# Coder-Yu/QRec

Measured on NVIDIA H100. Metric: BPR triples/sec at d=64, higher is better.
Workload: dtype f32

## Files before the change

qrec_b200/csrc/bpr_kernels.cu:

```cuda
#include <cmath>

#include "common.h"
#include "device.cuh"
#include "lane_shape.h"
#include "philox.cuh"
#include "bpr_step.cuh"
#include "um_waves.cuh"

namespace {

using namespace qrec;
using namespace qrec::bpr;

template <typename T, int E>
__global__ void __launch_bounds__(256)
bpr_sgd_ordered_kernel(T* __restrict__ P, T* __restrict__ Q, int d, long long n,
                       const int* __restrict__ u, const int* __restrict__ i,
                       const int* __restrict__ j, const int* __restrict__ wu,
                       const int* __restrict__ wi, const int* __restrict__ wj, int* ver_p,
                       int* ver_q, unsigned long long* ticket, T lr, T reg_u, T reg_i,
                       double* loss) {
  const int lane = threadIdx.x & 31;
  double local_loss = 0.0;
  const T a_u = mul_rn(lr, reg_u), a_i = mul_rn(lr, reg_i);
  while (true) {
    unsigned long long k = 0;
    if (lane == 0) k = atomicAdd(ticket, 1ULL);
    k = __shfl_sync(0xffffffffu, k, 0);
    if (k >= (unsigned long long)n) break;
    const int uu = u[k], ii = i[k], jj = j[k];
    const int* vp = lane == 0 ? ver_p + uu : (lane == 1 ? ver_q + ii : ver_q + jj);
    const int need = lane == 0 ? wu[k] : (lane == 1 ? wi[k] : wj[k]);
    unsigned backoff = 8, polls = 0;
    while (true) {
      const int have = lane < 3 ? ld_acquire_gpu(vp) : need;
      if (__all_sync(0xffffffffu, have == need)) break;
      __nanosleep(backoff);
      if (backoff < 64) backoff <<= 1;
      if (++polls > (1u << 27)) __trap();
    }
    T* pr = P + (size_t)uu * d;
    T* qir = Q + (size_t)ii * d;
    T* qjr = Q + (size_t)jj * d;
    T p[E], qi[E], qj[E];
    T di = 0, dj = 0;
#pragma unroll
    for (int e = 0; e < E; ++e) {
      const int c = e * 32 + lane;
      if (c < d) {
        p[e] = __ldcg(pr + c);
        qi[e] = __ldcg(qir + c);
        qj[e] = __ldcg(qjr + c);
        di += p[e] * qi[e];
        dj += p[e] * qj[e];
      } else {
        p[e] = qi[e] = qj[e] = 0;
      }
    }
    di = warp_sum(di);
    dj = warp_sum(dj);
    const T s = sigmoid_full(sub_rn(di, dj));
    const T g = mul_rn(lr, sub_rn((T)1, s));
#pragma unroll
    for (int e = 0; e < E; ++e) {
      const int c = e * 32 + lane;
      if (c < d) {
        T pn, qin, qjn;
        bpr_update_parity(p[e], qi[e], qj[e], g, a_u, a_i, pn, qin, qjn);
        __stcg(pr + c, pn);
        __stcg(qir + c, qin);
        __stcg(qjr + c, qjn);
      }
    }
    __threadfence();
    __syncwarp();
    if (lane < 3) red_release_gpu_add(const_cast<int*>(vp), 1);
    if (lane == 0) local_loss += neg_log(s);
  }
  if (lane == 0 && local_loss != 0.0) atomicAdd(loss, local_loss);
}

template <int LPR, int VPL, int UNROLL>
__global__ void __launch_bounds__(256)
bpr_sgd_batch_kernel(float* __restrict__ P, float* __restrict__ Q, int nvec, long long n,
                     const int* __restrict__ u, const int* __restrict__ i,
                     const int* __restrict__ j, float lr, float reg_u, float reg_i,
                     double* loss) {
  constexpr int TPW = 32 / LPR;
  const int lane = threadIdx.x & 31;
  const int sub = lane / LPR, l = lane % LPR;
  const long long warp = ((long long)blockIdx.x * blockDim.x + threadIdx.x) >> 5;
  const long long nwarps = ((long long)gridDim.x * blockDim.x) >> 5;
  const int d = nvec * 4;
  const float a_u = lr * reg_u, a_i = lr * reg_i;
  float lsum = 0.f;

  for (long long base = warp * 32; base < n; base += nwarps * 32) {
    const long long k = base + lane;
    int mu = 0, mi = 0, mj = 0;
    if (k < n) {
      mu = __ldg(u + k);
      mi = __ldg(i + k);
      mj = __ldg(j + k);
    }
    const int cnt = (n - base) < 32 ? (int)(n - base) : 32;
    for (int s0 = 0; s0 < cnt; s0 += TPW * UNROLL) {
      float4 p[UNROLL][VPL], qi[UNROLL][VPL], qj[UNROLL][VPL];
      float* pr[UNROLL];
      float* qir[UNROLL];
      float* qjr[UNROLL];
      bool ok[UNROLL];
#pragma unroll
      for (int r = 0; r < UNROLL; ++r) {
        const int t = s0 + r * TPW + sub;
        const int uu = __shfl_sync(0xffffffffu, mu, t & 31);
        const int ii = __shfl_sync(0xffffffffu, mi, t & 31);
        const int jj = __shfl_sync(0xffffffffu, mj, t & 31);
        ok[r] = t < cnt;
        pr[r] = P + (size_t)uu * d + l * 4;
        qir[r] = Q + (size_t)ii * d + l * 4;
        qjr[r] = Q + (size_t)jj * d + l * 4;
#pragma unroll
        for (int v = 0; v < VPL; ++v) {
          if (ok[r] && (l + v * LPR) < nvec) {
            p[r][v] = *reinterpret_cast<const float4*>(pr[r] + v * LPR * 4);
            qi[r][v] = *reinterpret_cast<const float4*>(qir[r] + v * LPR * 4);
            qj[r][v] = *reinterpret_cast<const float4*>(qjr[r] + v * LPR * 4);
          } else {
            p[r][v] = qi[r][v] = qj[r][v] = make_float4(0.f, 0.f, 0.f, 0.f);
          }
        }
      }
#pragma unroll
      for (int r = 0; r < UNROLL; ++r) {
        float x = 0.f;
#pragma unroll
        for (int v = 0; v < VPL; ++v) x += dot4(p[r][v], qi[r][v]) - dot4(p[r][v], qj[r][v]);
        x = group_sum<LPR>(x);
        const float s = fast_sigmoid(x);
        const float g = lr * (1.0f - s);
        if (ok[r]) {
          if (l == 0) lsum += fast_neg_log(s);
#pragma unroll
          for (int v = 0; v < VPL; ++v) {
            if ((l + v * LPR) < nvec) {
              float4 dp, dqi, dqj;
              bpr_step4(p[r][v], qi[r][v], qj[r][v], g, a_u, a_i, dp, dqi, dqj);
              red_add_v4(pr[r] + v * LPR * 4, dp);
              red_add_v4(qir[r] + v * LPR * 4, dqi);
              red_add_v4(qjr[r] + v * LPR * 4, dqj);
            }
          }
        }
      }
    }
  }
  block_add_loss(lsum, loss);
}


template <int LPR>
__global__ void __launch_bounds__(256)
bpr_sgd_staged_kernel(float* __restrict__ P, int nvec, long long n, const int* __restrict__ u,
                      const int* __restrict__ pos_i, const int* __restrict__ pos_j,
                      const float* __restrict__ R, float* __restrict__ D, float lr, float reg_u,
                      float reg_i, double* loss) {
  constexpr int TPW = 32 / LPR;
  const int lane = threadIdx.x & 31;
  const int sub = lane / LPR, l = lane % LPR;
  const long long group = (((long long)blockIdx.x * blockDim.x + threadIdx.x) >> 5) * TPW + sub;
  const long long ngroups = (((long long)gridDim.x * blockDim.x) >> 5) * TPW;
  const int d = nvec * 4;
  const float a_u = lr * reg_u, a_i = lr * reg_i;
  float lsum = 0.f;
  const long long rounds = (n + ngroups - 1) / ngroups;
  for (long long it = 0; it < rounds; ++it) {
    const long long k = it * ngroups + group;
    const bool ok = k < n && l < nvec;
    float4 p = make_float4(0.f, 0.f, 0.f, 0.f), qi = p, qj = p;
    float* pr = nullptr;
    size_t oi = 0, oj = 0;
    if (ok) {
      pr = P + (size_t)__ldg(u + k) * d + l * 4;
      oi = (size_t)__ldg(pos_i + k) * d + l * 4;
      oj = (size_t)__ldg(pos_j + k) * d + l * 4;
      p = *reinterpret_cast<const float4*>(pr);
      qi = __ldg(reinterpret_cast<const float4*>(R + oi));
      qj = __ldg(reinterpret_cast<const float4*>(R + oj));
    }
    float x = dot4(p, qi) - dot4(p, qj);
    x = group_sum<LPR>(x);
    const float s = fast_sigmoid(x);
    const float g = lr * (1.0f - s);
    if (ok) {
      if (l == 0) lsum += fast_neg_log(s);
      float4 dp, dqi, dqj;
      bpr_step4(p, qi, qj, g, a_u, a_i, dp, dqi, dqj);
      red_add_v4(pr, dp);
      *reinterpret_cast<float4*>(D + oi) = dqi;
      *reinterpret_cast<float4*>(D + oj) = dqj;
    }
  }
  block_add_loss(lsum, loss);
}


template <int UNROLL, int TMA_MASK>
__global__ void __launch_bounds__(256)
bpr_sgd_batch_tma_kernel(float* __restrict__ P, float* __restrict__ Q, long long n,
                         const int* __restrict__ u, const int* __restrict__ i,
                         const int* __restrict__ j, float lr, float reg_u, float reg_i,
                         double* loss) {
  constexpr int LPR = 16, TPW = 2, D = 64;
  constexpr int ROWS = ((TMA_MASK >> 0) & 1) + ((TMA_MASK >> 1) & 1) + ((TMA_MASK >> 2) & 1);
  constexpr int SLOT_P = 0, SLOT_I = (TMA_MASK & 1), SLOT_J = (TMA_MASK & 1) + ((TMA_MASK >> 1) & 1);
  constexpr int SLOT_FLOATS = UNROLL * TPW * ROWS * D;
  extern __shared__ __align__(128) float stage[];
  const int lane = threadIdx.x & 31, wib = threadIdx.x >> 5;
  const int sub = lane / LPR, l = lane % LPR;
  const long long warp = ((long long)blockIdx.x * blockDim.x + threadIdx.x) >> 5;
  const long long nwarps = ((long long)gridDim.x * blockDim.x) >> 5;
  const float a_u = lr * reg_u, a_i = lr * reg_i;
  float* my_stage = stage + (size_t)wib * 2 * SLOT_FLOATS;
  float lsum = 0.f;
  int buf = 0;

  for (long long base = warp * 32; base < n; base += nwarps * 32) {
    const long long k = base + lane;
    int mu = 0, mi = 0, mj = 0;
    if (k < n) {
      mu = __ldg(u + k);
      mi = __ldg(i + k);
      mj = __ldg(j + k);
    }
    const int cnt = (n - base) < 32 ? (int)(n - base) : 32;
    for (int s0 = 0; s0 < cnt; s0 += TPW * UNROLL) {
      float4 p[UNROLL], qi[UNROLL], qj[UNROLL];
      int uu[UNROLL], ii[UNROLL], jj[UNROLL];
      bool ok[UNROLL];
#pragma unroll
      for (int r = 0; r < UNROLL; ++r) {
        const int t = s0 + r * TPW + sub;
        uu[r] = __shfl_sync(0xffffffffu, mu, t & 31);
        ii[r] = __shfl_sync(0xffffffffu, mi, t & 31);
        jj[r] = __shfl_sync(0xffffffffu, mj, t & 31);
        ok[r] = t < cnt;
        if (ok[r]) {
          p[r] = *reinterpret_cast<const float4*>(P + (size_t)uu[r] * D + l * 4);
          qi[r] = *reinterpret_cast<const float4*>(Q + (size_t)ii[r] * D + l * 4);
          qj[r] = *reinterpret_cast<const float4*>(Q + (size_t)jj[r] * D + l * 4);
        } else {
          p[r] = qi[r] = qj[r] = make_float4(0.f, 0.f, 0.f, 0.f);
        }
      }
      if (l < 3) asm volatile("cp.async.bulk.wait_group.read 1;" ::: "memory");
      __syncwarp();
      float* slot = my_stage + (size_t)buf * SLOT_FLOATS;
#pragma unroll
      for (int r = 0; r < UNROLL; ++r) {
        float x = dot4(p[r], qi[r]) - dot4(p[r], qj[r]);
        x = group_sum<LPR>(x);
        const float s = fast_sigmoid(x);
        const float g = lr * (1.0f - s);
        if (ok[r]) {
          if (l == 0) lsum += fast_neg_log(s);
          float4 dp, dqi, dqj;
          bpr_step4(p[r], qi[r], qj[r], g, a_u, a_i, dp, dqi, dqj);
          float* trip = slot + (size_t)(r * TPW + sub) * ROWS * D;
          if (TMA_MASK & 1) *reinterpret_cast<float4*>(trip + SLOT_P * D + l * 4) = dp;
          else red_add_v4(P + (size_t)uu[r] * D + l * 4, dp);
          if (TMA_MASK & 2) *reinterpret_cast<float4*>(trip + SLOT_I * D + l * 4) = dqi;
          else red_add_v4(Q + (size_t)ii[r] * D + l * 4, dqi);
          if (TMA_MASK & 4) *reinterpret_cast<float4*>(trip + SLOT_J * D + l * 4) = dqj;
          else red_add_v4(Q + (size_t)jj[r] * D + l * 4, dqj);
        }
      }
      asm volatile("fence.proxy.async.shared::cta;" ::: "memory");
      __syncwarp();
      if (l < 3 && ((TMA_MASK >> l) & 1)) {
        const int srow = (l == 0) ? SLOT_P : (l == 1 ? SLOT_I : SLOT_J);
#pragma unroll
        for (int r = 0; r < UNROLL; ++r) {
          if (ok[r]) {
            float* dst = (l == 0) ? (P + (size_t)uu[r] * D) : (Q + (size_t)(l == 1 ? ii[r] : jj[r]) * D);
            const float* src = slot + (size_t)(r * TPW + sub) * ROWS * D + srow * D;
            asm volatile("cp.reduce.async.bulk.global.shared::cta.bulk_group.add.f32 [%0], [%1], %2;" ::"l"(dst),
                         "r"((uint32_t)__cvta_generic_to_shared(src)), "n"(D * 4)
                         : "memory");
          }
        }
        asm volatile("cp.async.bulk.commit_group;" ::: "memory");
      }
      buf ^= 1;
    }
  }
  if (l < 3) asm volatile("cp.async.bulk.wait_group 0;" ::: "memory");
  block_add_loss(lsum, loss);
}


constexpr int UM_STAGE_FLOATS = 2 * 4 * 64;
constexpr int UM_STAGE_GROUPS = 16;
constexpr int UM_STAGE_SMEM = UM_STAGE_GROUPS * 2 * (UM_STAGE_FLOATS * 4 + 8);

__device__ __forceinline__ void bulk_row_load(float* smem_dst, const float* gsrc, uint64_t* bar) {
  asm volatile("cp.async.bulk.shared::cluster.global.mbarrier::complete_tx::bytes [%0], [%1], 256, [%2];"
               ::"r"(smem_u32(smem_dst)), "l"(gsrc), "r"(smem_u32(bar)) : "memory");
}

template <int LPR, int G, bool FULL, bool SAMPLE, bool SIG, bool TMA>
__device__ __forceinline__ void
usermajor_epoch(float* __restrict__ P, float* __restrict__ Q, const float* __restrict__ Qr, int nvec, long long n,
                const int* __restrict__ wave_user, const long long* __restrict__ rowptr, const int* __restrict__ i,
                const int* __restrict__ j, float lr, float reg_u, float reg_i, double* loss, FusedSampler fs,
                long long trip_off, const uint32_t* __restrict__ rated_sig) {
  static_assert(!TMA || (LPR == 16 && G == 4 && FULL), "the TMA fetch is laid out for d = 64, G = 4");
  constexpr int GPW = 32 / LPR;
  const int lane = threadIdx.x & 31;
  const int sub = lane / LPR, l = lane % LPR;
  const unsigned gmask = (LPR == 32) ? 0xffffffffu : (((1u << LPR) - 1u) << (sub * LPR));
  const int group = (int)((blockIdx.x * blockDim.x + threadIdx.x) >> 5) * GPW + sub;
  const int ngroups = (int)((gridDim.x * blockDim.x) >> 5) * GPW;
  const int d = FULL ? LPR * 4 : nvec * 4;
  const bool act = FULL ? true : (l < nvec);
  const float a_u = lr * reg_u, a_i = lr * reg_i;
  const float one_m_au = 1.0f - a_u, one_m_ai = 1.0f - a_i;
  float lsum = 0.f;
  qrec::pdl_launch_dependents();
  bool waited = false;
  float* stage = nullptr;
  uint64_t* bar = nullptr;
  uint32_t phase0 = 0, phase1 = 0;
  if constexpr (TMA) {
    extern __shared__ __align__(128) unsigned char smem_raw[];
    float* stage_all = reinterpret_cast<float*>(smem_raw);
    uint64_t* bars = reinterpret_cast<uint64_t*>(stage_all + UM_STAGE_GROUPS * 2 * UM_STAGE_FLOATS);
    const int g_in_cta = (threadIdx.x >> 5) * GPW + sub;
    stage = stage_all + (size_t)g_in_cta * 2 * UM_STAGE_FLOATS;
    bar = bars + g_in_cta * 2;
    if (l == 0) { mbar_init(bar, 1); mbar_init(bar + 1, 1); }
    asm volatile("fence.mbarrier_init.release.cluster;" ::: "memory");
    asm volatile("fence.proxy.async.shared::cta;" ::: "memory");
    __syncthreads();
  }
  const int ub = __ldg(wave_user + 1);
  for (int uu = __ldg(wave_user) + group; uu < ub; uu += ngroups) {
    long long lo = __ldg(rowptr + uu) - trip_off, hi = __ldg(rowptr + uu + 1) - trip_off;
    lo = lo > 0 ? lo : 0;
    hi = hi < n ? hi : n;
    if (lo >= hi) continue;
    float* prow = P + (size_t)uu * d + l * 4;
    float4 p = act ? *reinterpret_cast<const float4*>(prow) : make_float4(0.f, 0.f, 0.f, 0.f);
    long long rated_lo = 0, rated_hi = 0;
    if (SAMPLE) {
      rated_lo = __ldg(fs.rated_rowptr + uu);
      rated_hi = __ldg(fs.rated_rowptr + uu + 1);
    }
    for (long long base = lo; base < hi; base += LPR) {
      const int m = (hi - base) < LPR ? (int)(hi - base) : LPR;
      int mi = 0, mj = 0;
      if (l < m) {
        mi = __ldg(i + base + l);
        if (SAMPLE) {
          if (SIG)
            mj = qrec::sample_negative_sig(base + l + trip_off, fs.epoch, fs.seed_lo, fs.seed_hi, fs.num_items,
                                           fs.rated_cols, rated_lo, rated_hi,
                                           rated_sig + (size_t)uu * qrec::RATED_SIG_WORDS);
          else
            mj = qrec::sample_negative(base + l + trip_off, fs.epoch, fs.seed_lo, fs.seed_hi, fs.num_items, fs.rated_cols,
                                       rated_lo, rated_hi);
        } else {
          mj = __ldg(j + base + l);
        }
      }
      if (!waited) {
        qrec::pdl_wait();
        waited = true;
      }
      if (SAMPLE && l < m && fs.j_out != nullptr) fs.j_out[base + l] = mj;
      auto issue = [&](int t0) {
        const int src = sub * LPR + ((t0 + (l >> 1)) & (LPR - 1));
        const int idi = __shfl_sync(gmask, mi, src), idj = __shfl_sync(gmask, mj, src);
        const int rows_now = 2 * ((m - t0) < G ? (m - t0) : G);
        uint64_t* bb = bar + ((t0 / G) & 1);
        if (l == 0) mbar_expect_tx(bb, 256u * rows_now);
        __syncwarp(gmask);
        if (l < rows_now) bulk_row_load(stage + ((t0 / G) & 1) * UM_STAGE_FLOATS + l * 64, Qr + (size_t)((l & 1) ? idj : idi) * d, bb);
      };
      if constexpr (TMA) issue(0);
      for (int t0 = 0; t0 < m; t0 += G) {
        const float* slot = nullptr;
        if constexpr (TMA) {
          if (t0 + G < m) issue(t0 + G);
          const int s = (t0 / G) & 1;
          mbar_wait(bar + s, s ? phase1 : phase0);
          if (s) phase1 ^= 1u; else phase0 ^= 1u;
          slot = stage + s * UM_STAGE_FLOATS;
        }
        float4 qi[G], qj[G];
        int ri[G], rj[G];
#pragma unroll
        for (int f = 0; f < G; ++f) {
          ri[f] = __shfl_sync(gmask, mi, sub * LPR + ((t0 + f) & (LPR - 1)));
          rj[f] = __shfl_sync(gmask, mj, sub * LPR + ((t0 + f) & (LPR - 1)));
          if (t0 + f < m && act) {
            if constexpr (TMA) {
              qi[f] = *reinterpret_cast<const float4*>(slot + (2 * f) * 64 + l * 4);
              qj[f] = *reinterpret_cast<const float4*>(slot + (2 * f + 1) * 64 + l * 4);
            } else {
              qi[f] = qrec::ldg_no_l1_v4(reinterpret_cast<const float4*>(Qr + (size_t)ri[f] * d + l * 4));
              qj[f] = qrec::ldg_no_l1_v4(reinterpret_cast<const float4*>(Qr + (size_t)rj[f] * d + l * 4));
            }
          } else {
            qi[f] = qj[f] = make_float4(0.f, 0.f, 0.f, 0.f);
          }
        }
        if constexpr (TMA) __syncwarp(gmask);
#pragma unroll
        for (int f = 0; f < G; ++f) {
          if (t0 + f < m) {
            float x = dot4(p, qi[f]) - dot4(p, qj[f]);
            x = group_sum<LPR>(x, gmask);
            const float s = fast_sigmoid(x);
            const float g = lr * (1.0f - s);
            if (l == 0) lsum += fast_neg_log(s);
            if (act) {
              float4 dqi, dqj;
              bpr_step4_inplace(p, qi[f], qj[f], g, one_m_au, g * one_m_ai, a_i, dqi, dqj);
              red_add_v4(Q + (size_t)ri[f] * d + l * 4, dqi);
              red_add_v4(Q + (size_t)rj[f] * d + l * 4, dqj);
            }
          }
        }
      }
    }
    if (act) {
      const float4 p0 = __ldcg(reinterpret_cast<const float4*>(prow));
      red_add_v4(prow, make_float4(p.x - p0.x, p.y - p0.y, p.z - p0.z, p.w - p0.w));
    }
  }
  if (!waited) qrec::pdl_wait();
  block_add_loss(lsum, loss);
}

template <int LPR, int G, bool FULL, bool SAMPLE, int MINB = 3, bool SIG = false>
__global__ void __launch_bounds__(256, MINB)
bpr_sgd_usermajor_kernel(float* __restrict__ P, float* __restrict__ Q, const float* __restrict__ Qr, int nvec, long long n,
                         const int* __restrict__ wave_user, const long long* __restrict__ rowptr,
                         const int* __restrict__ i, const int* __restrict__ j, float lr, float reg_u, float reg_i,
                         double* loss, FusedSampler fs, long long trip_off, const uint32_t* __restrict__ rated_sig) {
  usermajor_epoch<LPR, G, FULL, SAMPLE, SIG, false>(P, Q, Qr, nvec, n, wave_user, rowptr, i, j, lr, reg_u, reg_i, loss, fs,
                                                    trip_off, rated_sig);
}

__global__ void __launch_bounds__(256, 3)
bpr_sgd_usermajor_tma_kernel(float* __restrict__ P, float* __restrict__ Q, const float* __restrict__ Qr, int nvec,
                             long long n, const int* __restrict__ wave_user, const long long* __restrict__ rowptr,
                             const int* __restrict__ i, const int* __restrict__ j, float lr, float reg_u, float reg_i,
                             double* loss, FusedSampler fs, long long trip_off, const uint32_t* __restrict__ rated_sig) {
  usermajor_epoch<16, 4, true, true, false, true>(P, Q, Qr, nvec, n, wave_user, rowptr, i, j, lr, reg_u, reg_i, loss, fs,
                                                  trip_off, rated_sig);
}

using UserMajorKernel = decltype(&bpr_sgd_usermajor_tma_kernel);

template <int LPR>
UserMajorKernel usermajor_kernel(int nvec, bool sample, bool sig) {
  if (nvec != LPR)
    return sample ? bpr_sgd_usermajor_kernel<LPR, 4, false, true> : bpr_sgd_usermajor_kernel<LPR, 4, false, false>;
  if (sig) return bpr_sgd_usermajor_kernel<LPR, 2, true, true, 4, true>;
  return sample ? bpr_sgd_usermajor_kernel<LPR, 2, true, true, 4> : bpr_sgd_usermajor_kernel<LPR, 4, true, false>;
}

constexpr int UM_SNAPSHOT_THREADS = 512, UM_SNAPSHOT_CTAS_PER_SM = 4;
__global__ void __launch_bounds__(UM_SNAPSHOT_THREADS, UM_SNAPSHOT_CTAS_PER_SM)
um_snapshot_kernel(const float4* __restrict__ Q, float4* __restrict__ Qr, long long n4) {
  const unsigned long long keep = qrec::l2_policy_evict_last();
  qrec::pdl_wait();
  qrec::pdl_launch_dependents();
  const long long stride = (long long)gridDim.x * blockDim.x;
  long long k = (long long)blockIdx.x * blockDim.x + threadIdx.x;
  for (; k + 3 * stride < n4; k += 4 * stride) {
    float4 v[4];
#pragma unroll
    for (int r = 0; r < 4; ++r) v[r] = qrec::ld_stream_v4(Q + k + r * stride, keep);
#pragma unroll
    for (int r = 0; r < 4; ++r) qrec::st_hint_v4(Qr + k + r * stride, v[r], keep);
  }
  for (; k < n4; k += stride) qrec::st_hint_v4(Qr + k, qrec::ld_stream_v4(Q + k, keep), keep);
}

__global__ void __launch_bounds__(256)
um_wave_table_kernel(const long long* __restrict__ rowptr, int n_users, long long n, long long trip_off,
                     long long wave_chunks, long long nwaves, int* __restrict__ wave_user) {
  const long long w = (long long)blockIdx.x * blockDim.x + threadIdx.x;
  if (w <= nwaves) wave_user[w] = um_wave_first_user(rowptr, n_users, n, trip_off, wave_chunks, w);
}

__global__ void __launch_bounds__(256)
rated_signature_kernel(int n_users, const long long* __restrict__ rowptr, const int* __restrict__ cols,
                       uint32_t* __restrict__ sig) {
  const int lane = threadIdx.x & 31;
  const long long warp = ((long long)blockIdx.x * blockDim.x + threadIdx.x) >> 5;
  const long long nwarps = ((long long)gridDim.x * blockDim.x) >> 5;
  for (long long uu = warp; uu < n_users; uu += nwarps) {
    const long long lo = __ldg(rowptr + uu), hi = __ldg(rowptr + uu + 1);
    for (long long e = lo + lane; e < hi; e += 32) {
      const int c = __ldg(cols + e);
      atomicOr(sig + (size_t)uu * qrec::RATED_SIG_WORDS + ((c >> 5) & (qrec::RATED_SIG_WORDS - 1)), 1u << (c & 31));
    }
  }
}

template <typename T>
__global__ void __launch_bounds__(256)
sumsq_kernel(const T* __restrict__ x, long long n, double* out) {
  double acc = 0.0;
  const long long tid = (long long)blockIdx.x * blockDim.x + threadIdx.x;
  const long long stride = (long long)gridDim.x * blockDim.x;
  if constexpr (sizeof(T) == 4) {
    const long long n4 = n >> 2;
    const float4* x4 = reinterpret_cast<const float4*>(x);
    for (long long k = tid; k < n4; k += stride) {
      const float4 v = __ldg(x4 + k);
      acc += (double)v.x * v.x + (double)v.y * v.y + (double)v.z * v.z + (double)v.w * v.w;
    }
    for (long long k = (n4 << 2) + tid; k < n; k += stride) acc += (double)x[k] * x[k];
  } else {
    for (long long k = tid; k < n; k += stride) acc += (double)x[k] * (double)x[k];
  }
  acc = warp_sum(acc);
  __shared__ double wsum[8];
  if ((threadIdx.x & 31) == 0) wsum[threadIdx.x >> 5] = acc;
  __syncthreads();
  if (threadIdx.x == 0) {
    double t = 0.0;
    for (int w = 0; w < (int)(blockDim.x >> 5); ++w) t += wsum[w];
    atomicAdd(out, t);
  }
}

template <typename T>
int launch_ordered(T* P, T* Q, int d, long long n, const int* u, const int* i, const int* j,
                   const int* wu, const int* wi, const int* wj, int* ver_p, int* ver_q,
                   unsigned long long* ticket, T lr, T reg_u, T reg_i, double* loss,
                   int n_warps, cudaStream_t st) {
  QREC_REQUIRE(P && Q && loss && ticket && ver_p && ver_q, "bpr_sgd_ordered: null pointer");
  QREC_REQUIRE(d >= 1 && d <= 256, "bpr_sgd_ordered: d=%d unsupported (1..256)", d);
  QREC_REQUIRE(n >= 0, "bpr_sgd_ordered: n < 0");
  if (n == 0) return QREC_OK;
  QREC_REQUIRE(u && i && j && wu && wi && wj, "bpr_sgd_ordered: null index pointer");
  const int grid = n_warps > 0 ? capped_grid((n_warps + 7) / 8, 2) : sm_count() * 2;
  with_lane_elems(d, [&](auto e) {
    bpr_sgd_ordered_kernel<T, decltype(e)::E><<<grid, 256, 0, st>>>(P, Q, d, n, u, i, j, wu, wi, wj, ver_p, ver_q,
                                                                    ticket, lr, reg_u, reg_i, loss);
  });
  QREC_LAUNCH_CHECK();
  return QREC_OK;
}

}

namespace qrec {
int launch_bpr_batch(float* P, float* Q, int d, long long n, const int* u, const int* i,
                     const int* j, float lr, float reg_u, float reg_i, double* loss,
                     cudaStream_t st) {
  QREC_REQUIRE(P && Q && loss, "bpr_sgd_batch: null pointer");
  QREC_REQUIRE(d >= 4 && d <= 256 && (d % 4) == 0, "bpr_sgd_batch: d=%d unsupported (multiple of 4, 4..256)", d);
  QREC_REQUIRE(n >= 0, "bpr_sgd_batch: n < 0");
  if (n == 0) return QREC_OK;
  QREC_REQUIRE(u && i && j, "bpr_sgd_batch: null index pointer");
  const int nvec = d / 4;
  const long long warps_needed = (n + 31) / 32;
  const int grid = capped_grid((warps_needed + 7) / 8, 8);
  with_row_shape<256>(nvec, [&](auto s) {
    using S = decltype(s);
    bpr_sgd_batch_kernel<S::LPR, S::VPL, S::UNROLL><<<grid, 256, 0, st>>>(P, Q, nvec, n, u, i, j, lr, reg_u, reg_i,
                                                                          loss);
  });
  QREC_LAUNCH_CHECK();
  return QREC_OK;
}
}

extern "C" {

int qrec_bpr_sgd_ordered_f32(float* P, float* Q, int32_t d, int64_t n, const int32_t* u,
                             const int32_t* i, const int32_t* j, const int32_t* wu,
                             const int32_t* wi, const int32_t* wj, int32_t* ver_p,
                             int32_t* ver_q, unsigned long long* ticket, float lr, float reg_u,
                             float reg_i, double* loss, int32_t n_warps, void* stream) {
  return launch_ordered<float>(P, Q, d, n, u, i, j, wu, wi, wj, ver_p, ver_q, ticket, lr, reg_u,
                               reg_i, loss, n_warps, (cudaStream_t)stream);
}

int qrec_bpr_sgd_ordered_f64(double* P, double* Q, int32_t d, int64_t n, const int32_t* u,
                             const int32_t* i, const int32_t* j, const int32_t* wu,
                             const int32_t* wi, const int32_t* wj, int32_t* ver_p,
                             int32_t* ver_q, unsigned long long* ticket, double lr,
                             double reg_u, double reg_i, double* loss, int32_t n_warps, void* stream) {
  return launch_ordered<double>(P, Q, d, n, u, i, j, wu, wi, wj, ver_p, ver_q, ticket, lr, reg_u,
                                reg_i, loss, n_warps, (cudaStream_t)stream);
}

int qrec_bpr_sgd_batch_f32(float* P, float* Q, int32_t d, int64_t n, const int32_t* u,
                           const int32_t* i, const int32_t* j, float lr, float reg_u,
                           float reg_i, double* loss, void* stream) {
  return qrec::launch_bpr_batch(P, Q, d, n, u, i, j, lr, reg_u, reg_i, loss, (cudaStream_t)stream);
}

int qrec_bpr_sgd_batch_tma_f32(float* P, float* Q, int32_t d, int64_t n, const int32_t* u,
                               const int32_t* i, const int32_t* j, float lr, float reg_u,
                               float reg_i, double* loss, void* stream) {
  QREC_REQUIRE(P && Q && loss, "qrec_bpr_sgd_batch_tma_f32: null pointer");
  QREC_REQUIRE(d == 64, "qrec_bpr_sgd_batch_tma_f32: only d=64 (got %d); use qrec_bpr_sgd_batch_f32", d);
  QREC_REQUIRE(n >= 0, "qrec_bpr_sgd_batch_tma_f32: n < 0");
  if (n == 0) return QREC_OK;
  QREC_REQUIRE(u && i && j, "qrec_bpr_sgd_batch_tma_f32: null index pointer");
  constexpr int UN = 4, MASK = 1;
  constexpr int smem = 8 * 2 * UN * 2 * 64 * 4;
  QREC_CUDA(allow_dynamic_smem((const void*)bpr_sgd_batch_tma_kernel<UN, MASK>, smem));
  const int grid = capped_grid(((n + 31) / 32 + 7) / 8, 2);
  bpr_sgd_batch_tma_kernel<UN, MASK><<<grid, 256, smem, (cudaStream_t)stream>>>(P, Q, n, u, i, j, lr, reg_u, reg_i, loss);
  QREC_LAUNCH_CHECK();
  return QREC_OK;
}

}

namespace qrec {
int launch_usermajor(float* P, float* Q, int32_t d, int32_t n_users, int64_t n, const int64_t* rowptr,
                     const int32_t* i, const int32_t* j, float lr, float reg_u, float reg_i, double* loss,
                     bool sample, const int64_t* rated_rowptr, const int32_t* rated_cols, int32_t num_items,
                     uint64_t seed, uint32_t epoch, int32_t* j_out, long long trip_off, cudaStream_t st,
                     const uint32_t* rated_sig, bool tma) {
  if (n <= 0) return QREC_OK;
  QREC_REQUIRE(num_items >= 1, "qrec user-major epoch: num_items=%d (the item table's rows) must be given", num_items);
  QREC_REQUIRE(!tma || (d == 64 && sample), "qrec user-major epoch: the TMA fetch needs d = 64 and fused sampling");
  FusedSampler fs = {reinterpret_cast<const long long*>(rated_rowptr), rated_cols, num_items, (uint32_t)seed,
                     (uint32_t)(seed >> 32), epoch, j_out};
  const int nvec = d / 4;
  const int lpr = row_lpr(nvec);
  const bool sig = sample && rated_sig != nullptr;
  const UserMajorKernel kernel =
      tma ? bpr_sgd_usermajor_tma_kernel
          : with_row_shape<128>(nvec, [&](auto s) { return usermajor_kernel<decltype(s)::LPR>(nvec, sample, sig); });
  const int smem = tma ? UM_STAGE_SMEM : 0;
  if (tma) QREC_CUDA(allow_dynamic_smem((const void*)kernel, smem));
  int occ = 3;
  if (cudaOccupancyMaxActiveBlocksPerMultiprocessor(&occ, kernel, 256, smem) != cudaSuccess || occ < 1) occ = 3;
  const long long per_block = 8 * (32 / lpr);
  const long long max_users = n < n_users ? n : n_users;
  const int grid = capped_grid((max_users + per_block - 1) / per_block, occ);
  const size_t q_bytes = (size_t)num_items * d * sizeof(float);
  const long long wave = um_wave_chunks(n, num_items, d);
  const long long nwaves = um_num_waves(n, wave);
  float* Qr = nullptr;
  int* wave_user = nullptr;
  QREC_CUDA(cudaMallocAsync(reinterpret_cast<void**>(&Qr), q_bytes, st));
  const int rc = [&]() -> int {
    QREC_CUDA(cudaMallocAsync(reinterpret_cast<void**>(&wave_user), sizeof(int) * (size_t)(nwaves + 1), st));
    um_wave_table_kernel<<<(unsigned)((nwaves + 256) / 256), 256, 0, st>>>(reinterpret_cast<const long long*>(rowptr), n_users,
                                                                          n, trip_off, wave, nwaves, wave_user);
    QREC_CUDA(cudaGetLastError());
    count_launch();
    cudaLaunchAttribute pdl;
    pdl.id = cudaLaunchAttributeProgrammaticStreamSerialization;
    pdl.val.programmaticStreamSerializationAllowed = 1;
    const auto launch = [&](auto* fn, dim3 g, dim3 b, size_t shm, bool chained, auto... args) {
      cudaLaunchConfig_t cfg = {};
      cfg.gridDim = g;
      cfg.blockDim = b;
      cfg.dynamicSmemBytes = shm;
      cfg.stream = st;
      cfg.attrs = chained ? &pdl : nullptr;
      cfg.numAttrs = chained ? 1 : 0;
      return cudaLaunchKernelEx(&cfg, fn, args...);
    };
    const long long n4 = (long long)(q_bytes / sizeof(float4));
    const int copy_grid = sm_count() * UM_SNAPSHOT_CTAS_PER_SM;
    for (long long w = 0; w < nwaves; ++w) {
      QREC_CUDA(launch(um_snapshot_kernel, dim3(copy_grid), dim3(UM_SNAPSHOT_THREADS), 0, w > 0,
                       reinterpret_cast<const float4*>(Q), reinterpret_cast<float4*>(Qr), n4));
      count_launch();
      QREC_CUDA(launch(kernel, dim3(grid), dim3(256), (size_t)smem, true, P, Q, static_cast<const float*>(Qr), nvec,
                       (long long)n, static_cast<const int*>(wave_user + w), reinterpret_cast<const long long*>(rowptr), i, j,
                       lr, reg_u, reg_i, loss, fs, trip_off, rated_sig));
      if (w + 1 < nwaves) count_launch();
    }
    return QREC_OK;
  }();
  if (wave_user != nullptr) QREC_CUDA(cudaFreeAsync(wave_user, st));
  QREC_CUDA(cudaFreeAsync(Qr, st));
  if (rc != QREC_OK) return rc;
  QREC_LAUNCH_CHECK();
  return QREC_OK;
}
}

extern "C" {

int qrec_bpr_sgd_usermajor_f32(float* P, float* Q, int32_t d, int32_t n_users, int64_t n, int32_t num_items,
                               const int64_t* rowptr, const int32_t* i, const int32_t* j, float lr, float reg_u, float reg_i,
                               double* loss, void* stream) {
  QREC_REQUIRE(P && Q && loss, "qrec_bpr_sgd_usermajor_f32: null pointer");
  QREC_REQUIRE(d >= 4 && d <= 128 && (d % 4) == 0, "qrec_bpr_sgd_usermajor_f32: d=%d unsupported (multiple of 4, 4..128)", d);
  QREC_REQUIRE(n_users >= 0 && n >= 0, "qrec_bpr_sgd_usermajor_f32: negative size");
  if (n_users == 0 || n == 0) return QREC_OK;
  QREC_REQUIRE(rowptr && i && j, "qrec_bpr_sgd_usermajor_f32: null index pointer");
  return qrec::launch_usermajor(P, Q, d, n_users, n, rowptr, i, j, lr, reg_u, reg_i, loss, false, nullptr, nullptr, num_items,
                                0, 0, nullptr, 0, (cudaStream_t)stream, nullptr, false);
}

int qrec_bpr_epoch_usermajor_f32(float* P, float* Q, int32_t d, int32_t n_users, int64_t n, const int64_t* rowptr,
                                 const int32_t* i, const int64_t* rated_rowptr, const int32_t* rated_cols,
                                 int32_t num_items, uint64_t seed, uint32_t epoch, int32_t* j_out, float lr,
                                 float reg_u, float reg_i, double* loss, void* stream) {
  QREC_REQUIRE(P && Q && loss, "qrec_bpr_epoch_usermajor_f32: null pointer");
  QREC_REQUIRE(d >= 4 && d <= 128 && (d % 4) == 0, "qrec_bpr_epoch_usermajor_f32: d=%d unsupported (multiple of 4, 4..128)", d);
  QREC_REQUIRE(n_users >= 0 && n >= 0 && num_items >= 1, "qrec_bpr_epoch_usermajor_f32: bad size");
  if (n_users == 0 || n == 0) return QREC_OK;
  QREC_REQUIRE(rowptr && i && rated_rowptr && rated_cols, "qrec_bpr_epoch_usermajor_f32: null index pointer");
  return qrec::launch_usermajor(P, Q, d, n_users, n, rowptr, i, nullptr, lr, reg_u, reg_i, loss, true, rated_rowptr,
                                rated_cols, num_items, seed, epoch, j_out, 0, (cudaStream_t)stream, nullptr, false);
}

int qrec_rated_signature_build(int32_t n_users, const int64_t* rated_rowptr, const int32_t* rated_cols,
                               uint32_t* sig, void* stream) {
  QREC_REQUIRE(n_users >= 0, "qrec_rated_signature_build: n_users < 0");
  if (n_users == 0) return QREC_OK;
  QREC_REQUIRE(rated_rowptr && rated_cols && sig, "qrec_rated_signature_build: null pointer");
  cudaStream_t st = (cudaStream_t)stream;
  QREC_CUDA(cudaMemsetAsync(sig, 0, (size_t)n_users * qrec::RATED_SIG_WORDS * sizeof(uint32_t), st));
  rated_signature_kernel<<<capped_grid(((long long)n_users + 7) / 8, 8), 256, 0, st>>>(n_users, reinterpret_cast<const long long*>(rated_rowptr),
                                                     rated_cols, sig);
  QREC_LAUNCH_CHECK();
  return QREC_OK;
}

int qrec_bpr_epoch_usermajor_sig_f32(float* P, float* Q, int32_t d, int32_t n_users, int64_t n, const int64_t* rowptr,
                                     const int32_t* i, const int64_t* rated_rowptr, const int32_t* rated_cols,
                                     const uint32_t* rated_sig, int32_t num_items, uint64_t seed, uint32_t epoch,
                                     int32_t* j_out, float lr, float reg_u, float reg_i, double* loss, void* stream) {
  QREC_REQUIRE(P && Q && loss, "qrec_bpr_epoch_usermajor_sig_f32: null pointer");
  QREC_REQUIRE(d == 16 || d == 32 || d == 64 || d == 128,
               "qrec_bpr_epoch_usermajor_sig_f32: d=%d unsupported (16, 32, 64 or 128); use qrec_bpr_epoch_usermajor_f32", d);
  QREC_REQUIRE(n_users >= 0 && n >= 0 && num_items >= 1, "qrec_bpr_epoch_usermajor_sig_f32: bad size");
  if (n_users == 0 || n == 0) return QREC_OK;
  QREC_REQUIRE(rowptr && i && rated_rowptr && rated_cols && rated_sig, "qrec_bpr_epoch_usermajor_sig_f32: null index pointer");
  return qrec::launch_usermajor(P, Q, d, n_users, n, rowptr, i, nullptr, lr, reg_u, reg_i, loss, true, rated_rowptr,
                                rated_cols, num_items, seed, epoch, j_out, 0, (cudaStream_t)stream, rated_sig, false);
}

int qrec_bpr_epoch_usermajor_tma_f32(float* P, float* Q, int32_t d, int32_t n_users, int64_t n, const int64_t* rowptr,
                                     const int32_t* i, const int64_t* rated_rowptr, const int32_t* rated_cols,
                                     int32_t num_items, uint64_t seed, uint32_t epoch, int32_t* j_out, float lr,
                                     float reg_u, float reg_i, double* loss, void* stream) {
  QREC_REQUIRE(P && Q && loss, "qrec_bpr_epoch_usermajor_tma_f32: null pointer");
  QREC_REQUIRE(d == 64, "qrec_bpr_epoch_usermajor_tma_f32: d=%d unsupported (64 only: one 256-byte bulk copy per row); use "
                        "qrec_bpr_epoch_usermajor_f32", d);
  QREC_REQUIRE(n_users >= 0 && n >= 0 && num_items >= 1, "qrec_bpr_epoch_usermajor_tma_f32: bad size");
  if (n_users == 0 || n == 0) return QREC_OK;
  QREC_REQUIRE(rowptr && i && rated_rowptr && rated_cols, "qrec_bpr_epoch_usermajor_tma_f32: null index pointer");
  QREC_REQUIRE((reinterpret_cast<uintptr_t>(Q) & 15) == 0, "qrec_bpr_epoch_usermajor_tma_f32: Q must be 16-byte aligned");
  return qrec::launch_usermajor(P, Q, d, n_users, n, rowptr, i, nullptr, lr, reg_u, reg_i, loss, true, rated_rowptr,
                                rated_cols, num_items, seed, epoch, j_out, 0, (cudaStream_t)stream, nullptr, true);
}

int qrec_bpr_sgd_staged_f32(float* P, int32_t d, int64_t n, const int32_t* u, const int32_t* pos_i,
                            const int32_t* pos_j, const float* R, float* D, float lr, float reg_u,
                            float reg_i, double* loss, void* stream) {
  QREC_REQUIRE(d >= 4 && d <= 128 && (d % 4) == 0, "qrec_bpr_sgd_staged_f32: d=%d unsupported (multiple of 4, 4..128)", d);
  QREC_REQUIRE(n >= 0, "qrec_bpr_sgd_staged_f32: n < 0");
  if (n == 0) return QREC_OK;
  QREC_REQUIRE(P && u && pos_i && pos_j && R && D && loss, "qrec_bpr_sgd_staged_f32: null pointer");
  const int nvec = d / 4;
  cudaStream_t st = (cudaStream_t)stream;
  with_row_shape<128>(nvec, [&](auto s) {
    constexpr int LPR = decltype(s)::LPR;
    const long long per_block = 8 * (32 / LPR);
    const int grid = capped_grid((n + per_block - 1) / per_block, 8);
    bpr_sgd_staged_kernel<LPR><<<grid, 256, 0, st>>>(P, nvec, n, u, pos_i, pos_j, R, D, lr, reg_u, reg_i, loss);
  });
  QREC_LAUNCH_CHECK();
  return QREC_OK;
}

int qrec_sumsq_f32(const float* x, int64_t n, double* out, void* stream) {
  QREC_REQUIRE(out && (x || n == 0) && n >= 0, "qrec_sumsq_f32: bad argument");
  if (n == 0) return QREC_OK;
  QREC_REQUIRE((reinterpret_cast<uintptr_t>(x) & 15) == 0, "qrec_sumsq_f32: x not 16-byte aligned");
  sumsq_kernel<float><<<capped_grid((n / 4 + 255) / 256 + 1, 8), 256, 0, (cudaStream_t)stream>>>(x, n, out);
  QREC_LAUNCH_CHECK();
  return QREC_OK;
}

int qrec_table_snapshot_f32(const float* src, float* dst, int64_t n, void* stream) {
  QREC_REQUIRE(n >= 0 && (n % 4) == 0, "qrec_table_snapshot_f32: n=%lld must be a multiple of 4", (long long)n);
  if (n == 0) return QREC_OK;
  QREC_REQUIRE(src && dst, "qrec_table_snapshot_f32: null pointer");
  QREC_REQUIRE(((reinterpret_cast<uintptr_t>(src) | reinterpret_cast<uintptr_t>(dst)) & 15) == 0,
               "qrec_table_snapshot_f32: src and dst must be 16-byte aligned");
  um_snapshot_kernel<<<sm_count() * UM_SNAPSHOT_CTAS_PER_SM, UM_SNAPSHOT_THREADS, 0, (cudaStream_t)stream>>>(reinterpret_cast<const float4*>(src),
                                                                                 reinterpret_cast<float4*>(dst), n / 4);
  QREC_LAUNCH_CHECK();
  return QREC_OK;
}

int qrec_sumsq_f64(const double* x, int64_t n, double* out, void* stream) {
  QREC_REQUIRE(out && (x || n == 0) && n >= 0, "qrec_sumsq_f64: bad argument");
  if (n == 0) return QREC_OK;
  sumsq_kernel<double><<<capped_grid((n + 255) / 256, 8), 256, 0, (cudaStream_t)stream>>>(x, n, out);
  QREC_LAUNCH_CHECK();
  return QREC_OK;
}

}
```

qrec_b200/csrc/device.cuh:

```cuda
#pragma once
#include <cstdint>

namespace qrec {

__device__ __forceinline__ void red_add_v4(float* addr, float4 v) {
  asm volatile("red.global.add.v4.f32 [%0], {%1, %2, %3, %4};" ::"l"(addr), "f"(v.x), "f"(v.y), "f"(v.z), "f"(v.w) : "memory");
}

__device__ __forceinline__ unsigned long long l2_policy_evict_last() {
  unsigned long long pol;
  asm volatile("createpolicy.fractional.L2::evict_last.b64 %0, 1.0;" : "=l"(pol));
  return pol;
}
__device__ __forceinline__ float4 ld_stream_v4(const float4* p, unsigned long long pol) {
  float4 v;
  asm volatile("ld.global.nc.L1::no_allocate.L2::cache_hint.v4.f32 {%0, %1, %2, %3}, [%4], %5;"
               : "=f"(v.x), "=f"(v.y), "=f"(v.z), "=f"(v.w) : "l"(p), "l"(pol));
  return v;
}
__device__ __forceinline__ void st_hint_v4(float4* p, float4 v, unsigned long long pol) {
  asm volatile("st.global.L2::cache_hint.v4.f32 [%0], {%1, %2, %3, %4}, %5;" ::"l"(p), "f"(v.x), "f"(v.y), "f"(v.z), "f"(v.w),
               "l"(pol) : "memory");
}
__device__ __forceinline__ float4 ldg_no_l1_v4(const float4* p) {
  float4 v;
  asm volatile("ld.global.nc.L1::no_allocate.v4.f32 {%0, %1, %2, %3}, [%4];"
               : "=f"(v.x), "=f"(v.y), "=f"(v.z), "=f"(v.w) : "l"(p));
  return v;
}

__device__ __forceinline__ void pdl_wait() { asm volatile("griddepcontrol.wait;" ::: "memory"); }
__device__ __forceinline__ void pdl_launch_dependents() { asm volatile("griddepcontrol.launch_dependents;" ::: "memory"); }

__device__ __forceinline__ float dot4(float4 a, float4 b) { return a.x * b.x + a.y * b.y + a.z * b.z + a.w * b.w; }

__device__ __forceinline__ void fma4(float4& acc, float s, float4 x) {
  acc.x = fmaf(s, x.x, acc.x); acc.y = fmaf(s, x.y, acc.y);
  acc.z = fmaf(s, x.z, acc.z); acc.w = fmaf(s, x.w, acc.w);
}

template <typename T>
__device__ __forceinline__ T warp_sum(T v) {
#pragma unroll
  for (int o = 16; o > 0; o >>= 1) v += __shfl_xor_sync(0xffffffffu, v, o);
  return v;
}

template <int LPR>
__device__ __forceinline__ float group_sum(float v, unsigned mask = 0xffffffffu) {
#pragma unroll
  for (int o = LPR / 2; o > 0; o >>= 1) v += __shfl_xor_sync(mask, v, o);
  return v;
}

__device__ __forceinline__ float fast_sigmoid(float x) { return __fdividef(1.0f, 1.0f + __expf(-x)); }
__device__ __forceinline__ float fast_neg_log(float s) { return -__logf(s); }

__device__ __forceinline__ int ld_acquire_gpu(const int* p) {
  int v;
  asm volatile("ld.acquire.gpu.global.s32 %0, [%1];" : "=r"(v) : "l"(p) : "memory");
  return v;
}
__device__ __forceinline__ void red_release_gpu_add(int* p, int v) {
  asm volatile("red.release.gpu.global.add.s32 [%0], %1;" ::"l"(p), "r"(v) : "memory");
}

__device__ __forceinline__ void block_add_loss(float lsum, double* loss) {
  __shared__ float wsum[8];
  lsum = warp_sum(lsum);
  if ((threadIdx.x & 31) == 0) wsum[threadIdx.x >> 5] = lsum;
  __syncthreads();
  if (threadIdx.x == 0) {
    double t = 0.0;
    for (int w = 0; w < (int)(blockDim.x >> 5); ++w) t += (double)wsum[w];
    if (t != 0.0) atomicAdd(loss, t);
  }
}

__device__ __forceinline__ uint32_t smem_u32(const void* p) { return (uint32_t)__cvta_generic_to_shared(p); }

__device__ __forceinline__ void mbar_init(uint64_t* bar, uint32_t count) {
  asm volatile("mbarrier.init.shared::cta.b64 [%0], %1;" ::"r"(smem_u32(bar)), "r"(count));
}
__device__ __forceinline__ void mbar_expect_tx(uint64_t* bar, uint32_t bytes) {
  asm volatile("mbarrier.arrive.expect_tx.shared::cta.b64 _, [%0], %1;" ::"r"(smem_u32(bar)), "r"(bytes) : "memory");
}
__device__ __forceinline__ void mbar_arrive(uint64_t* bar) {
  asm volatile("mbarrier.arrive.shared::cta.b64 _, [%0];" ::"r"(smem_u32(bar)) : "memory");
}
__device__ __forceinline__ bool mbar_try_wait(uint64_t* bar, uint32_t parity) {
  uint32_t ok;
  asm volatile(
      "{\n\t.reg .pred p;\n\t"
      "mbarrier.try_wait.parity.shared::cta.b64 p, [%1], %2;\n\t"
      "selp.u32 %0, 1, 0, p;\n\t}"
      : "=r"(ok)
      : "r"(smem_u32(bar)), "r"(parity)
      : "memory");
  return ok != 0;
}
__device__ __forceinline__ void mbar_wait(uint64_t* bar, uint32_t parity) {
  for (uint32_t spins = 0;; ++spins) {
    if (mbar_try_wait(bar, parity)) return;
    if (spins > (1u << 22)) __trap();
  }
}

}
```

qrec_b200/csrc/philox.cuh:

```cuda
#pragma once
#include <cstdint>

namespace qrec {

__device__ __forceinline__ void philox4x32_10(uint32_t c0, uint32_t c1, uint32_t c2, uint32_t c3,
                                              uint32_t k0, uint32_t k1, uint32_t out[4]) {
  constexpr uint32_t M0 = 0xD2511F53u, M1 = 0xCD9E8D57u, W0 = 0x9E3779B9u, W1 = 0xBB67AE85u;
#pragma unroll
  for (int r = 0; r < 10; ++r) {
    const uint32_t hi0 = __umulhi(M0, c0), lo0 = M0 * c0;
    const uint32_t hi1 = __umulhi(M1, c2), lo1 = M1 * c2;
    const uint32_t n0 = hi1 ^ c1 ^ k0, n1 = lo1, n2 = hi0 ^ c3 ^ k1, n3 = lo0;
    c0 = n0; c1 = n1; c2 = n2; c3 = n3;
    k0 += W0; k1 += W1;
  }
  out[0] = c0; out[1] = c1; out[2] = c2; out[3] = c3;
}

__device__ __forceinline__ int sample_negative(long long k, uint32_t epoch, uint32_t seed_lo, uint32_t seed_hi,
                                               int num_items, const int* __restrict__ cols, long long lo0,
                                               long long hi0) {
  const bool saturated = (hi0 - lo0) >= (long long)num_items;
  uint32_t attempt = 0;
  while (true) {
    uint32_t w[4];
    philox4x32_10((uint32_t)k, (uint32_t)((unsigned long long)k >> 32), attempt, epoch, seed_lo, seed_hi, w);
    const int j = (int)(((unsigned long long)w[0] * (unsigned long long)(uint32_t)num_items) >> 32);
    if (saturated) return j;
    long long lo = lo0, hi = hi0;
    bool hit = false;
    while (lo < hi) {
      const long long mid = (lo + hi) >> 1;
      const int c = __ldg(cols + mid);
      if (c < j) lo = mid + 1;
      else if (c > j) hi = mid;
      else { hit = true; break; }
    }
    if (!hit) return j;
    ++attempt;
  }
}

constexpr int RATED_SIG_WORDS = 16;
__device__ __forceinline__ int sample_negative_sig(long long k, uint32_t epoch, uint32_t seed_lo, uint32_t seed_hi,
                                                   int num_items, const int* __restrict__ cols, long long lo0,
                                                   long long hi0, const uint32_t* __restrict__ sig) {
  const bool saturated = (hi0 - lo0) >= (long long)num_items;
  uint32_t attempt = 0;
  while (true) {
    uint32_t w[4];
    philox4x32_10((uint32_t)k, (uint32_t)((unsigned long long)k >> 32), attempt, epoch, seed_lo, seed_hi, w);
    const int j = (int)(((unsigned long long)w[0] * (unsigned long long)(uint32_t)num_items) >> 32);
    if (saturated) return j;
    const uint32_t word = __ldg(sig + ((j >> 5) & (RATED_SIG_WORDS - 1)));
    if (((word >> (j & 31)) & 1u) == 0u) return j;
    long long lo = lo0, hi = hi0;
    bool hit = false;
    while (lo < hi) {
      const long long mid = (lo + hi) >> 1;
      const int c = __ldg(cols + mid);
      if (c < j) lo = mid + 1;
      else if (c > j) hi = mid;
      else { hit = true; break; }
    }
    if (!hit) return j;
    ++attempt;
  }
}

struct FusedSampler {
  const long long* rated_rowptr;
  const int* rated_cols;
  int num_items;
  uint32_t seed_lo, seed_hi, epoch;
  int* j_out;
};

}
```

Before: 3.211 billion.

## Prefetch next chunk's item indices and negatives into shared memory via cp.async

```diff
diff --git a/qrec_b200/csrc/bpr_kernels.cu b/qrec_b200/csrc/bpr_kernels.cu
--- a/qrec_b200/csrc/bpr_kernels.cu
+++ b/qrec_b200/csrc/bpr_kernels.cu
@@ -319,7 +319,7 @@
   const int lane = threadIdx.x & 31;
   const int sub = lane / LPR, l = lane % LPR;
   const unsigned gmask = (LPR == 32) ? 0xffffffffu : (((1u << LPR) - 1u) << (sub * LPR));
-  const int group = (int)((blockIdx.x * blockDim.x + threadIdx.x) >> 5) * GPW + sub;
+  const int group = ((int)(threadIdx.x >> 5) * GPW + sub) * (int)gridDim.x + (int)blockIdx.x;
   const int ngroups = (int)((gridDim.x * blockDim.x) >> 5) * GPW;
   const int d = FULL ? LPR * 4 : nvec * 4;
   const bool act = FULL ? true : (l < nvec);
@@ -343,6 +343,10 @@
     asm volatile("fence.proxy.async.shared::cta;" ::: "memory");
     __syncthreads();
   }
+  __shared__ int2 um_idx[2][256];
+  __shared__ uint32_t um_sig_word[SIG ? 256 : 1];
+  const int gl0 = threadIdx.x - l;
+  uint32_t& sig_w = um_sig_word[SIG ? threadIdx.x : 0];
   const int ub = __ldg(wave_user + 1);
   for (int uu = __ldg(wave_user) + group; uu < ub; uu += ngroups) {
     long long lo = __ldg(rowptr + uu) - trip_off, hi = __ldg(rowptr + uu + 1) - trip_off;
@@ -356,36 +360,54 @@
       rated_lo = __ldg(fs.rated_rowptr + uu);
       rated_hi = __ldg(fs.rated_rowptr + uu + 1);
     }
+    const uint32_t* sig_u = SIG ? rated_sig + (size_t)uu * qrec::RATED_SIG_WORDS : nullptr;
+    auto fetch = [&](long long b, int sl) {
+      int2* slot = um_idx[sl] + gl0;
+      if (l < hi - b) {
+        qrec::cp_async_4(&slot[l].x, i + b + l);
+        if (SAMPLE) {
+          const int j0 = qrec::negative_candidate(b + l + trip_off, 0, fs.epoch, fs.seed_lo, fs.seed_hi, fs.num_items);
+          slot[l].y = j0;
+          if (SIG) qrec::cp_async_4(&sig_w, qrec::rated_sig_word_ptr(sig_u, j0));
+        } else {
+          qrec::cp_async_4(&slot[l].y, j + b + l);
+        }
+      }
+    };
+    auto resolve = [&](long long b, int sl) {
+      int2* slot = um_idx[sl] + gl0;
+      if (l < hi - b) {
+        qrec::cp_async_wait_all();
+        if (SAMPLE) {
+          if (SIG)
+            slot[l].y = qrec::sample_negative_sig_from(b + l + trip_off, fs.epoch, fs.seed_lo, fs.seed_hi, fs.num_items,
+                                                       fs.rated_cols, rated_lo, rated_hi, sig_u, slot[l].y, sig_w);
+          else
+            slot[l].y = qrec::sample_negative_from(b + l + trip_off, fs.epoch, fs.seed_lo, fs.seed_hi, fs.num_items,
+                                                   fs.rated_cols, rated_lo, rated_hi, slot[l].y);
+        }
+      }
+    };
+    int cur = 0;
+    fetch(lo, 0);
+    resolve(lo, 0);
+    __syncwarp(gmask);
     for (long long base = lo; base < hi; base += LPR) {
       const int m = (hi - base) < LPR ? (int)(hi - base) : LPR;
-      int mi = 0, mj = 0;
-      if (l < m) {
-        mi = __ldg(i + base + l);
-        if (SAMPLE) {
-          if (SIG)
-            mj = qrec::sample_negative_sig(base + l + trip_off, fs.epoch, fs.seed_lo, fs.seed_hi, fs.num_items,
-                                           fs.rated_cols, rated_lo, rated_hi,
-                                           rated_sig + (size_t)uu * qrec::RATED_SIG_WORDS);
-          else
-            mj = qrec::sample_negative(base + l + trip_off, fs.epoch, fs.seed_lo, fs.seed_hi, fs.num_items, fs.rated_cols,
-                                       rated_lo, rated_hi);
-        } else {
-          mj = __ldg(j + base + l);
-        }
-      }
+      const int2* mine = um_idx[cur] + gl0;
+      const bool ahead = base + LPR < hi;
       if (!waited) {
         qrec::pdl_wait();
         waited = true;
       }
-      if (SAMPLE && l < m && fs.j_out != nullptr) fs.j_out[base + l] = mj;
+      if (SAMPLE && l < m && fs.j_out != nullptr) fs.j_out[base + l] = mine[l].y;
       auto issue = [&](int t0) {
-        const int src = sub * LPR + ((t0 + (l >> 1)) & (LPR - 1));
-        const int idi = __shfl_sync(gmask, mi, src), idj = __shfl_sync(gmask, mj, src);
+        const int2 e = mine[(t0 + (l >> 1)) & (LPR - 1)];
         const int rows_now = 2 * ((m - t0) < G ? (m - t0) : G);
         uint64_t* bb = bar + ((t0 / G) & 1);
         if (l == 0) mbar_expect_tx(bb, 256u * rows_now);
         __syncwarp(gmask);
-        if (l < rows_now) bulk_row_load(stage + ((t0 / G) & 1) * UM_STAGE_FLOATS + l * 64, Qr + (size_t)((l & 1) ? idj : idi) * d, bb);
+        if (l < rows_now) bulk_row_load(stage + ((t0 / G) & 1) * UM_STAGE_FLOATS + l * 64, Qr + (size_t)((l & 1) ? e.y : e.x) * d, bb);
       };
       if constexpr (TMA) issue(0);
       for (int t0 = 0; t0 < m; t0 += G) {
@@ -401,8 +423,9 @@
         int ri[G], rj[G];
 #pragma unroll
         for (int f = 0; f < G; ++f) {
-          ri[f] = __shfl_sync(gmask, mi, sub * LPR + ((t0 + f) & (LPR - 1)));
-          rj[f] = __shfl_sync(gmask, mj, sub * LPR + ((t0 + f) & (LPR - 1)));
+          const int2 e = mine[(t0 + f) & (LPR - 1)];
+          ri[f] = e.x;
+          rj[f] = e.y;
           if (t0 + f < m && act) {
             if constexpr (TMA) {
               qi[f] = *reinterpret_cast<const float4*>(slot + (2 * f) * 64 + l * 4);
@@ -432,12 +455,15 @@
             }
           }
         }
-      }
-    }
-    if (act) {
-      const float4 p0 = __ldcg(reinterpret_cast<const float4*>(prow));
-      red_add_v4(prow, make_float4(p.x - p0.x, p.y - p0.y, p.z - p0.z, p.w - p0.w));
-    }
+        if (ahead) {
+          if (t0 == 0) fetch(base + LPR, cur ^ 1);
+          if (t0 + G >= m) resolve(base + LPR, cur ^ 1);
+        }
+      }
+      __syncwarp(gmask);
+      cur ^= 1;
+    }
+    if (act) *reinterpret_cast<float4*>(prow) = p;
   }
   if (!waited) qrec::pdl_wait();
   block_add_loss(lsum, loss);
diff --git a/qrec_b200/csrc/device.cuh b/qrec_b200/csrc/device.cuh
--- a/qrec_b200/csrc/device.cuh
+++ b/qrec_b200/csrc/device.cuh
@@ -106,4 +106,9 @@
   }
 }
 
+__device__ __forceinline__ void cp_async_4(void* smem_dst, const void* gsrc) {
+  asm volatile("cp.async.ca.shared.global [%0], [%1], 4;" ::"r"(smem_u32(smem_dst)), "l"(gsrc) : "memory");
 }
+__device__ __forceinline__ void cp_async_wait_all() { asm volatile("cp.async.wait_all;" ::: "memory"); }
+
+}
diff --git a/qrec_b200/csrc/philox.cuh b/qrec_b200/csrc/philox.cuh
--- a/qrec_b200/csrc/philox.cuh
+++ b/qrec_b200/csrc/philox.cuh
@@ -41,31 +41,59 @@
   }
 }
 
+__device__ __forceinline__ int negative_candidate(long long k, uint32_t attempt, uint32_t epoch, uint32_t seed_lo,
+                                                  uint32_t seed_hi, int num_items) {
+  uint32_t w[4];
+  philox4x32_10((uint32_t)k, (uint32_t)((unsigned long long)k >> 32), attempt, epoch, seed_lo, seed_hi, w);
+  return (int)(((unsigned long long)w[0] * (unsigned long long)(uint32_t)num_items) >> 32);
+}
+
+__device__ __forceinline__ bool rated_contains(const int* __restrict__ cols, long long lo, long long hi, int j) {
+  while (lo < hi) {
+    const long long mid = (lo + hi) >> 1;
+    const int c = __ldg(cols + mid);
+    if (c < j) lo = mid + 1;
+    else if (c > j) hi = mid;
+    else return true;
+  }
+  return false;
+}
+
+__device__ __forceinline__ int sample_negative_from(long long k, uint32_t epoch, uint32_t seed_lo, uint32_t seed_hi,
+                                                    int num_items, const int* __restrict__ cols, long long lo0,
+                                                    long long hi0, int j0) {
+  if ((hi0 - lo0) >= (long long)num_items) return j0;
+  int j = j0;
+  for (uint32_t attempt = 1; rated_contains(cols, lo0, hi0, j); ++attempt)
+    j = negative_candidate(k, attempt, epoch, seed_lo, seed_hi, num_items);
+  return j;
+}
+
 constexpr int RATED_SIG_WORDS = 16;
+__device__ __forceinline__ const uint32_t* rated_sig_word_ptr(const uint32_t* sig, int j) {
+  return sig + ((j >> 5) & (RATED_SIG_WORDS - 1));
+}
+
+__device__ __forceinline__ int sample_negative_sig_from(long long k, uint32_t epoch, uint32_t seed_lo, uint32_t seed_hi,
+                                                        int num_items, const int* __restrict__ cols, long long lo0,
+                                                        long long hi0, const uint32_t* __restrict__ sig, int j0,
+                                                        uint32_t word0) {
+  if ((hi0 - lo0) >= (long long)num_items) return j0;
+  int j = j0;
+  uint32_t word = word0;
+  for (uint32_t attempt = 1; ((word >> (j & 31)) & 1u) != 0u && rated_contains(cols, lo0, hi0, j); ++attempt) {
+    j = negative_candidate(k, attempt, epoch, seed_lo, seed_hi, num_items);
+    word = __ldg(rated_sig_word_ptr(sig, j));
+  }
+  return j;
+}
+
 __device__ __forceinline__ int sample_negative_sig(long long k, uint32_t epoch, uint32_t seed_lo, uint32_t seed_hi,
                                                    int num_items, const int* __restrict__ cols, long long lo0,
                                                    long long hi0, const uint32_t* __restrict__ sig) {
-  const bool saturated = (hi0 - lo0) >= (long long)num_items;
-  uint32_t attempt = 0;
-  while (true) {
-    uint32_t w[4];
-    philox4x32_10((uint32_t)k, (uint32_t)((unsigned long long)k >> 32), attempt, epoch, seed_lo, seed_hi, w);
-    const int j = (int)(((unsigned long long)w[0] * (unsigned long long)(uint32_t)num_items) >> 32);
-    if (saturated) return j;
-    const uint32_t word = __ldg(sig + ((j >> 5) & (RATED_SIG_WORDS - 1)));
-    if (((word >> (j & 31)) & 1u) == 0u) return j;
-    long long lo = lo0, hi = hi0;
-    bool hit = false;
-    while (lo < hi) {
-      const long long mid = (lo + hi) >> 1;
-      const int c = __ldg(cols + mid);
-      if (c < j) lo = mid + 1;
-      else if (c > j) hi = mid;
-      else { hit = true; break; }
-    }
-    if (!hit) return j;
-    ++attempt;
-  }
+  const int j0 = negative_candidate(k, 0, epoch, seed_lo, seed_hi, num_items);
+  return sample_negative_sig_from(k, epoch, seed_lo, seed_hi, num_items, cols, lo0, hi0, sig, j0,
+                                  __ldg(rated_sig_word_ptr(sig, j0)));
 }
 
 struct FusedSampler {
```

Result: faster. 3.274 billion, median of 6 (+2.0%).
